# GTEC-UDC/roskfpos

Hardware: AMD Instinct MI355X
Metric: EKF predict+update steps/s at 65536 tags x 8 anchors; RMS pos err vs CPU ref (higher is better)
Workload: dtype f64 arithmetic; f64 state and covariance, f32/int32 measurements in HBM (KFPOS_STORE_MIXED)

## Files before the change

roskfpos_amd/csrc/kfpos_core.h:

```cpp
#ifndef KFPOS_CORE_H
#define KFPOS_CORE_H

#include <math.h>
#include <stdint.h>

#ifndef KFPOS_HD
#define KFPOS_HD
#endif
#define KFPOS_FN KFPOS_HD inline __attribute__((always_inline))
#if defined(__clang__)
#define KFPOS_UNROLL _Pragma("unroll")
#define KFPOS_NOUNROLL _Pragma("nounroll")
#else
#define KFPOS_UNROLL
#define KFPOS_NOUNROLL
#endif

#if defined(__HIP_DEVICE_COMPILE__)
#define KFPOS_WAVE_ALL(pred) (__all((pred) ? 1 : 0) != 0)
#else
#define KFPOS_WAVE_ALL(pred) (pred)
#endif
#if defined(__HIP_DEVICE_COMPILE__)
#define KFPOS_WAVE_ANY(pred) (__builtin_amdgcn_ballot_w64(pred) != 0)
#else
#define KFPOS_WAVE_ANY(pred) (pred)
#endif

namespace kfpos {

enum : uint32_t {
    ST_UPDATE_SKIPPED = 0x01u,
    ST_ML_FALLBACK    = 0x02u,
    ST_FEW_RANGES     = 0x04u,
    ST_ML_INIT        = 0x08u,
    ST_NOT_STARTED    = 0x10u,
    ST_NONFINITE      = 0x20u,
    ST_SKIPPED        = 0x40u,
};
enum : uint32_t { FL_STARTED = 1u, FL_HAS_IMU = 2u };

KFPOS_FN uint32_t pack_status(uint32_t flags, int gain_iters, int ml_iters, int ignored) {
    const uint32_t g = gain_iters > 255 ? 255u : (uint32_t)gain_iters;
    const uint32_t m = ml_iters > 255 ? 255u : (uint32_t)ml_iters;
    return flags | (g << 8) | (m << 16) | ((uint32_t)(ignored + 1) << 24);
}

KFPOS_FN double kf_rcp(double x) {
#if defined(__HIP_DEVICE_COMPILE__)
    double y = __builtin_amdgcn_rcp(x);
    double e = __builtin_fma(-x, y, 1.0);
    y = __builtin_fma(y, e, y);
    e = __builtin_fma(-x, y, 1.0);
    return __builtin_fma(y, e, y);
#else
    return 1.0 / x;
#endif
}
KFPOS_FN double kf_fma(double a, double b, double c) {
#if defined(__HIP_DEVICE_COMPILE__)
    return __builtin_fma(a, b, c);
#else
    return a * b + c;
#endif
}
KFPOS_FN int kf_opaque_zero() {
    int z = 0;
#if defined(__HIP_DEVICE_COMPILE__)
    asm volatile("" : "+v"(z));
#endif
    return z;
}
KFPOS_FN void kf_pin(double &v) {
#if defined(__HIP_DEVICE_COMPILE__)
    asm volatile("" : "+v"(v));
#else
    (void)v;
#endif
}
KFPOS_FN int kf_ctz64(uint64_t m) {
#if defined(__HIP_DEVICE_COMPILE__)
    return __ffsll((unsigned long long)m) - 1;
#else
    return __builtin_ctzll(m);
#endif
}
KFPOS_FN double kf_rsqrt(double x) {
#if defined(__HIP_DEVICE_COMPILE__)
    double y = __builtin_amdgcn_rsq(x);
    const double h = 0.5 * x;
    double e = __builtin_fma(-h * y, y, 0.5);
    y = __builtin_fma(y, e, y);
    e = __builtin_fma(-h * y, y, 0.5);
    return __builtin_fma(y, e, y);
#else
    return 1.0 / sqrt(x);
#endif
}
KFPOS_FN void kf_sqrt_rsqrt(double x, double &d, double &invd) {
#if defined(__HIP_DEVICE_COMPILE__)
    invd = kf_rsqrt(x);
    const double s = x * invd;
    d = __builtin_fma(__builtin_fma(-s, s, x) * 0.5, invd, s);
#else
    d = sqrt(x);
    invd = 1.0 / d;
#endif
}

KFPOS_FN void kf_sqrt_rsqrt_sweep(double x, double &d, double &invd) {
#if defined(__HIP_DEVICE_COMPILE__)
    double y = __builtin_amdgcn_rsq(x);
    const double e = __builtin_fma(-(0.5 * x) * y, y, 0.5);
    y = __builtin_fma(y, e, y);
    const double s = x * y;
    d = __builtin_fma(__builtin_fma(-s, s, x) * 0.5, y, s);
    invd = y;
#else
    d = sqrt(x);
    invd = 1.0 / d;
#endif
}

KFPOS_FN double kf_mm_to_m(int32_t mm) {
#if defined(__HIP_DEVICE_COMPILE__)
    const double x = (double)mm;
    const double q = x * 0.001;
    const double r = __builtin_fma(-q, 1000.0, x);
    return __builtin_fma(r, 0.001, q);
#else
    return (double)mm / 1000;
#endif
}

KFPOS_FN bool rel_change_below(double cost, double c, double tol) {
    const double lhs = fabs(cost - c), rhs = tol * cost;
    const bool clear = cost > 0.0 && fabs(lhs - rhs) > 1e-13 * rhs;
    if (KFPOS_WAVE_ALL(clear)) return lhs < rhs;
    return lhs / cost < tol;
}

KFPOS_FN bool rel_change_below_voted(double cost, double c, double tol) {
    const double lhs = fabs(cost - c), rhs = tol * cost;
    const bool clear = cost > 0.0 && fabs(lhs - rhs) > 1e-13 * rhs;
    bool below = lhs < rhs;
    if (KFPOS_WAVE_ANY(!clear)) below = lhs / cost < tol;
    return below;
}

KFPOS_FN bool rel_change_above(double cost, double c, double tol) {
    const double lhs = fabs(cost - c), rhs = tol * cost;
    const bool clear = cost > 0.0 && fabs(lhs - rhs) > 1e-13 * rhs;
    if (KFPOS_WAVE_ALL(clear)) return lhs > rhs;
    return lhs / cost > tol;
}

KFPOS_FN double stdmax(double a, double b) { return (a < b) ? b : a; }

template <int N, bool SYMM>
struct Cov {
    static constexpr int SZ = SYMM ? N * (N + 1) / 2 : N * N;
    double a[SZ];
    KFPOS_HD static constexpr int idx(int i, int j) {
        return SYMM ? (i <= j ? i * N - i * (i - 1) / 2 + (j - i) : j * N - j * (j - 1) / 2 + (i - j))
                    : i * N + j;
    }
    KFPOS_HD double operator()(int i, int j) const { return a[idx(i, j)]; }
    KFPOS_HD double &operator()(int i, int j) { return a[idx(i, j)]; }
};

struct Params {
    const double *anchors;
    int n_anchors;
    double accel_noise, jolt, cost_threshold;
    int ignore_worst, top_n, use_init_pos;
    int ml_variant = 0;
    int use_fixed_height, imu_fixed_cov_acc, imu_fixed_cov_w;
    double px4_height, px4_arm_p1, px4_arm_p2, px4_cov_vel, px4_cov_gyro_z;
    double imu_cov_acc, imu_cov_w, mag_offset, mag_cov;
    const double *pair_anchor_tab = nullptr;
    bool pair9 = false;
};

KFPOS_FN double sym3_cofactors(const double h[6], double c[6]) {
    c[0] = h[3] * h[5] - h[4] * h[4];
    c[1] = h[2] * h[4] - h[1] * h[5];
    c[2] = h[1] * h[4] - h[2] * h[3];
    c[3] = h[0] * h[5] - h[2] * h[2];
    c[4] = h[1] * h[2] - h[0] * h[4];
    c[5] = h[0] * h[3] - h[1] * h[1];
    return h[0] * c[0] + h[1] * c[1] + h[2] * c[2];
}
KFPOS_FN double gen3_adjugate(const double m[9], double adj[9]) {
    adj[0] = m[4] * m[8] - m[5] * m[7];
    adj[1] = m[2] * m[7] - m[1] * m[8];
    adj[2] = m[1] * m[5] - m[2] * m[4];
    adj[3] = m[5] * m[6] - m[3] * m[8];
    adj[4] = m[0] * m[8] - m[2] * m[6];
    adj[5] = m[2] * m[3] - m[0] * m[5];
    adj[6] = m[3] * m[7] - m[4] * m[6];
    adj[7] = m[1] * m[6] - m[0] * m[7];
    adj[8] = m[0] * m[4] - m[1] * m[3];
    return m[0] * adj[0] + m[1] * adj[3] + m[2] * adj[6];
}

template <int N, int K>
KFPOS_FN void gauss_solve(const double *a, const double *b, double *x) {
    double r[N][N + K];
    KFPOS_UNROLL
    for (int i = 0; i < N; ++i) {
        KFPOS_UNROLL
        for (int j = 0; j < N; ++j) r[i][j] = a[N * i + j];
        KFPOS_UNROLL
        for (int k = 0; k < K; ++k) r[i][N + k] = b[K * i + k];
    }
    KFPOS_UNROLL
    for (int c = 0; c < N; ++c) {
        KFPOS_UNROLL
        for (int i = c + 1; i < N; ++i) {
            const bool sw = fabs(r[i][c]) > fabs(r[c][c]);
            KFPOS_UNROLL
            for (int k = c; k < N + K; ++k) {
                const double tc = r[c][k], ti = r[i][k];
                r[c][k] = sw ? ti : tc;
                r[i][k] = sw ? tc : ti;
            }
        }
        const double ip = 1.0 / r[c][c];
        KFPOS_UNROLL
        for (int i = c + 1; i < N; ++i) {
            const double f = r[i][c] * ip;
            KFPOS_UNROLL
            for (int k = c + 1; k < N + K; ++k) r[i][k] -= f * r[c][k];
        }
// ... 47 lines not shown
    KFPOS_HD void setW(int a, double v) { w[a * stride] = v; }
    KFPOS_HD double Rdyn(int a) const { return r[a * stride]; }
    KFPOS_HD double Edyn(int a) const { return e[a * stride]; }
    KFPOS_HD void setWdyn(int a, double v) { w[a * stride] = v; }
};
template <int N>
struct StaticScratch : Scratch {
    static constexpr int NA = N;
    static constexpr int CHUNK = N > 8 ? 8 : 0;
};
template <int N>
struct StaticScratchF {
    static constexpr int NA = N;
    static constexpr int CHUNK = N > 8 ? 8 : 0;
    static constexpr bool COOP = false;
    double *r, *w;
    float *e;
    int stride;
    KFPOS_HD double R(int a) const { return r[a * stride]; }
    KFPOS_HD double E(int a) const { return (double)e[a * stride]; }
    KFPOS_HD double W(int a) const { return w[a * stride]; }
    KFPOS_HD void setW(int a, double v) { w[a * stride] = v; }
    KFPOS_HD double Rdyn(int a) const { return r[a * stride]; }
    KFPOS_HD double Edyn(int a) const { return (double)e[a * stride]; }
    KFPOS_HD void setWdyn(int a, double v) { w[a * stride] = v; }
};
template <int N>
struct RegScratch {
    static constexpr int NA = N;
    static constexpr int CHUNK = 0;
    static constexpr bool COOP = false;
    double r[N], e[N], w[N];
    KFPOS_HD double R(int a) const { return r[a]; }
    KFPOS_HD double E(int a) const { return e[a]; }
    KFPOS_HD double W(int a) const { return w[a]; }
    KFPOS_HD void setW(int a, double v) { w[a] = v; }
    KFPOS_HD double Rdyn(int a) const {
        double v = 0.0;
        KFPOS_UNROLL
        for (int k = 0; k < N; ++k) v = (k == a) ? r[k] : v;
        return v;
    }
    KFPOS_HD double Edyn(int a) const {
        double v = 1.0;
        KFPOS_UNROLL
        for (int k = 0; k < N; ++k) v = (k == a) ? e[k] : v;
        return v;
    }
    KFPOS_HD void setWdyn(int a, double v) {
        KFPOS_UNROLL
        for (int k = 0; k < N; ++k) w[k] = (k == a) ? v : w[k];
    }
};
struct CoopScratch {
    static constexpr int NA = 1;
    static constexpr int CHUNK = 0;
    static constexpr bool COOP = true;
    double r, e, w;
    double bx, by, bz;
    KFPOS_HD double R(int) const { return r; }
    KFPOS_HD double E(int) const { return e; }
    KFPOS_HD double W(int) const { return w; }
    KFPOS_HD void setW(int, double v) { w = v; }
    KFPOS_HD double Rdyn(int) const { return 0.0; }
    KFPOS_HD double Edyn(int) const { return 1.0; }
    KFPOS_HD void setWdyn(int, double) {}
};

template <class SC>
KFPOS_FN void anchor_of(const SC &sc, const Params &pr, int a, double &bx, double &by, double &bz) {
    if constexpr (SC::COOP) {
        bx = sc.bx; by = sc.by; bz = sc.bz;
    } else {
        bx = pr.anchors[3 * a]; by = pr.anchors[3 * a + 1]; bz = pr.anchors[3 * a + 2];
    }
}

#if defined(__HIP_DEVICE_COMPILE__)
KFPOS_FN double dpp_exchange(double v, int ctrl_tag) {
    const int lo = __double2loint(v), hi = __double2hiint(v);
    int plo, phi;
    if (ctrl_tag == 0) {
        plo = __builtin_amdgcn_mov_dpp(lo, 0xB1, 0xF, 0xF, true);
        phi = __builtin_amdgcn_mov_dpp(hi, 0xB1, 0xF, 0xF, true);
    } else if (ctrl_tag == 1) {
        plo = __builtin_amdgcn_mov_dpp(lo, 0x4E, 0xF, 0xF, true);
        phi = __builtin_amdgcn_mov_dpp(hi, 0x4E, 0xF, 0xF, true);
    } else {
        plo = __builtin_amdgcn_mov_dpp(lo, 0x141, 0xF, 0xF, true);
        phi = __builtin_amdgcn_mov_dpp(hi, 0x141, 0xF, 0xF, true);
    }
    return __hiloint2double(phi, plo);
}
#endif
template <class SC>
KFPOS_FN double group_sum(const SC &, double v) {
    if constexpr (SC::COOP) {
#if defined(__HIP_DEVICE_COMPILE__)
        v += dpp_exchange(v, 0);
        v += dpp_exchange(v, 1);
        v += dpp_exchange(v, 2);
#endif
    }
    return v;
}

// ... 36 lines not shown
```

roskfpos_amd/csrc/kfpos_core_imu9.h:

```cpp
#ifndef KFPOS_CORE_IMU9_H
#define KFPOS_CORE_IMU9_H

namespace kfpos {

constexpr double INFO_FORM_MIN_PIVOT = 1e-7;

struct Tag9 {
    double pos[3], vel[3];
    Cov<9, true> P;
};
struct Imu {
    bool has;
    double acc[3];
    double *ci;
    int ci_stride;
    KFPOS_HD double Wi(int k) const { return ci[(6 + k) * ci_stride]; }
};

KFPOS_FN void imu_whitener(const double s[9], double *ci, int ci_stride) {
    double c00, c11, c22, i00, i11, i22;
    kf_sqrt_rsqrt(s[0], c00, i00);
    const double c10 = s[3] * i00, c20 = s[6] * i00;
    kf_sqrt_rsqrt(s[4] - c10 * c10, c11, i11);
    const double c21 = (s[7] - c20 * c10) * i11;
    kf_sqrt_rsqrt(s[8] - c20 * c20 - c21 * c21, c22, i22);
    const double i10 = -c10 * i00 * i11;
    const double i21 = -c21 * i11 * i22;
    const double i20 = -(c20 * i00 + c21 * i10) * i22;
    ci[0] = i00; ci[ci_stride] = i10; ci[2 * ci_stride] = i20; ci[3 * ci_stride] = i11; ci[4 * ci_stride] = i21;
    ci[5 * ci_stride] = i22;
    double *wi = ci + 6 * ci_stride;
    wi[0] = i00 * i00 + i10 * i10 + i20 * i20;
    wi[ci_stride] = i10 * i11 + i20 * i21;
    wi[2 * ci_stride] = i20 * i22;
    wi[3 * ci_stride] = i11 * i11 + i21 * i21;
    wi[4 * ci_stride] = i21 * i22;
    wi[5 * ci_stride] = i22 * i22;
}

KFPOS_FN void predict9(Cov<9, true> &P, double t, double jolt) {
    const double c = t * t / 2;
    KFPOS_UNROLL
    for (int i = 0; i < 3; ++i) {
        KFPOS_UNROLL
        for (int j = i; j < 3; ++j) {
            const double xpp = P(i, j) + t * P(3 + i, j) + c * P(6 + i, j);
            const double xpv = P(i, 3 + j) + t * P(3 + i, 3 + j) + c * P(6 + i, 3 + j);
            const double xpa = P(i, 6 + j) + t * P(3 + i, 6 + j) + c * P(6 + i, 6 + j);
            P(i, j) = xpp + t * xpv + c * xpa;
        }
    }
    KFPOS_UNROLL
    for (int i = 0; i < 3; ++i) {
        KFPOS_UNROLL
        for (int j = 0; j < 3; ++j) {
            const double xpv = P(i, 3 + j) + t * P(3 + i, 3 + j) + c * P(6 + i, 3 + j);
            const double xpa = P(i, 6 + j) + t * P(3 + i, 6 + j) + c * P(6 + i, 6 + j);
            P(i, 3 + j) = xpv + t * xpa;
        }
    }
    KFPOS_UNROLL
    for (int i = 0; i < 3; ++i) {
        KFPOS_UNROLL
        for (int j = 0; j < 3; ++j) P(i, 6 + j) = P(i, 6 + j) + t * P(3 + i, 6 + j) + c * P(6 + i, 6 + j);
    }
    KFPOS_UNROLL
    for (int i = 0; i < 3; ++i) {
        KFPOS_UNROLL
        for (int j = i; j < 3; ++j) {
// ... 548 lines not shown
        iekf9_sweep4(p, r4, w4, bb, sw);
        other.c = dpp_exchange(sw.c, 0);
        KFPOS_UNROLL
        for (int k = 0; k < 6; ++k) other.m[k] = dpp_exchange(sw.m[k], 0);
        KFPOS_UNROLL
        for (int k = 0; k < 3; ++k) other.u[k] = dpp_exchange(sw.u[k], 0);
        sweep9_add(sw, other);
        iekf9_spread_reads();
        const bool more = iekf9_pass<DIAG, false>(xh, pk, ci, tol, sw, ct, co);
        act = more && co.gain_iters < max_steps;
    }
    const bool owner = (m >> lane) & 1ull;
    const int rank = __popcll(m & ((1ull << lane) - 1ull));
    const int from4 = (owner ? 2 * rank : lane) << 2;
    KFPOS_UNROLL
    for (int k = 0; k < 6; ++k) {
        const double a = lane_pull(ct.wl[k], from4), b = lane_pull(co.mrlast[k], from4);
        if (owner) { it.wl[k] = a; o.mrlast[k] = b; }
    }
    KFPOS_UNROLL
    for (int k = 0; k < 3; ++k) {
        const double a = lane_pull(co.dlast[k], from4);
        if (owner) o.dlast[k] = a;
    }
    const double cst = lane_pull(ct.cost, from4);
    const int gi = __builtin_amdgcn_ds_bpermute(from4, co.gain_iters);
    if (owner) { it.cost = cst; o.gain_iters = gi; }
}
template <bool DIAG, bool ALLIMU, bool ACC0>
KFPOS_FN void iekf9_pairs_held(uint64_t m, const double xhat[9], const double *binv, int binv_stride,
                               const RegScratch<8> &sc, const Params &pr, const Imu &imu, int max_steps, double tol,
                               Iekf9Iter &it, Iekf9Out &o) {
    const int lane = (int)__builtin_amdgcn_mbcnt_hi(~0u, __builtin_amdgcn_mbcnt_lo(~0u, 0u));
    const int g = lane >> 1;
    const bool h = lane & 1;
    const int n_surv = __popcll(m);
    bool act = g < n_surv;
    const int src = nth_set_bit(m, act ? g : 0);
    const int src4 = src << 2;
    Imu ci;
    ci.ci = imu.ci + (src - lane);
    ci.ci_stride = imu.ci_stride;
    Iekf9Parked pk;
    iekf9_fetch<false, DIAG, false>(binv + (src - lane), binv_stride, ci, pk);
    double xh[9];
    KFPOS_UNROLL
    for (int k = 0; k < 3; ++k) {
        xh[k] = lane_pull(xhat[k], src4);
        xh[3 + k] = 0.0;
        xh[6 + k] = ACC0 ? 0.0 : lane_pull(xhat[6 + k], src4);
    }
    Iekf9Iter ct;
    KFPOS_UNROLL
    for (int k = 0; k < 6; ++k) { ct.ve[k] = lane_pull(it.ve[k], src4); ct.wl[k] = 0.0; }
    ct.qd = lane_pull(it.qd, src4);
    ct.cost = lane_pull(it.cost, src4);
    Iekf9Out co;
    KFPOS_UNROLL
    for (int k = 0; k < 6; ++k) co.mrlast[k] = 0.0;
    KFPOS_UNROLL
    for (int k = 0; k < 3; ++k) co.dlast[k] = 0.0;
    co.gain_iters = __builtin_amdgcn_ds_bpermute(src4, o.gain_iters);
    ci.has = ALLIMU || __builtin_amdgcn_ds_bpermute(src4, imu.has ? 1 : 0) != 0;
    KFPOS_UNROLL
    for (int k = 0; k < 3; ++k) ci.acc[k] = lane_pull(imu.acc[k], src4);
    double r4[4], w4[4], bb[12];
    KFPOS_UNROLL
    for (int k = 0; k < 4; ++k) {
        const double r0 = lane_pull(sc.r[k], src4), r1 = lane_pull(sc.r[4 + k], src4);
        const double w0 = lane_pull(sc.w[k], src4), w1 = lane_pull(sc.w[4 + k], src4);
        r4[k] = h ? r1 : r0;
        w4[k] = h ? w1 : w0;
    }
    KFPOS_UNROLL
    for (int k = 0; k < 12; ++k) {
        bb[k] = h ? pr.anchors[12 + k] : pr.anchors[k];
        kf_pin(bb[k]);
    }
    KFPOS_UNROLL
    for (int k = 0; k < 21; ++k) kf_pin(pk.binv[k]);
    KFPOS_UNROLL
    for (int k = 0; k < 6; ++k) {
        if (!DIAG || k == 0 || k == 3 || k == 5) kf_pin(pk.wi[k]);
    }
    __builtin_amdgcn_s_waitcnt(0xC07F);
    while (act) {
        const double p[3] = {xh[0] + ct.ve[0], xh[1] + ct.ve[1], xh[2] + ct.ve[2]};
        Sweep9 sw, other;
        iekf9_sweep4(p, r4, w4, bb, sw);
        other.c = dpp_exchange(sw.c, 0);
        KFPOS_UNROLL
        for (int k = 0; k < 6; ++k) other.m[k] = dpp_exchange(sw.m[k], 0);
        KFPOS_UNROLL
        for (int k = 0; k < 3; ++k) other.u[k] = dpp_exchange(sw.u[k], 0);
        sweep9_add(sw, other);
        const bool more = iekf9_pass<DIAG, ALLIMU>(xh, pk, ci, tol, sw, ct, co);
        act = more && co.gain_iters < max_steps;
    }
    const bool owner = (m >> lane) & 1ull;
    const int rank = __popcll(m & ((1ull << lane) - 1ull));
    const int from4 = (owner ? 2 * rank : lane) << 2;
    const int gi = __builtin_amdgcn_ds_bpermute(from4, co.gain_iters);
    double back[16];
    KFPOS_UNROLL
    for (int k = 0; k < 6; ++k) { back[k] = lane_pull(ct.wl[k], from4); back[6 + k] = lane_pull(co.mrlast[k], from4); }
    KFPOS_UNROLL
    for (int k = 0; k < 3; ++k) back[12 + k] = lane_pull(co.dlast[k], from4);
    back[15] = lane_pull(ct.cost, from4);
    const bool moved = owner & (gi != o.gain_iters);
    KFPOS_UNROLL
    for (int k = 0; k < 6; ++k) { it.wl[k] = moved ? back[k] : it.wl[k]; o.mrlast[k] = moved ? back[6 + k] : o.mrlast[k]; }
    KFPOS_UNROLL
    for (int k = 0; k < 3; ++k) o.dlast[k] = moved ? back[12 + k] : o.dlast[k];
    it.cost = moved ? back[15] : it.cost;
    o.gain_iters = moved ? gi : o.gain_iters;
}
#endif

template <bool DIAG, bool ALLIMU, bool RANGING, bool ACC0 = false, bool HOLD = true, bool SETTLE = false,
          bool TAIL = false, class SC>
KFPOS_FN void iekf9_info(const double xhat[9], const double *binv, int binv_stride, SC &sc, const Params &pr,
                         const Imu &imu, int max_steps, double tol, Iekf9Out &o) {
    Iekf9Iter it;
    KFPOS_UNROLL
    for (int k = 0; k < 6; ++k) { it.ve[k] = 0.0; it.wl[k] = 0.0; o.mrlast[k] = 0.0; }
    it.qd = 0.0;
    it.cost = 1e20;
    o.dlast[0] = o.dlast[1] = o.dlast[2] = 0.0;
    o.gain_iters = 0;
// ... 283 lines not shown
```

roskfpos_amd/csrc/kfpos_core_ml.h:

```cpp
#ifndef KFPOS_CORE_ML_H
#define KFPOS_CORE_ML_H

namespace kfpos {

template <class SC>
KFPOS_FN void ml_sweep(const double p[3], const SC &sc, const Params &pr, uint64_t drop,
                              double &cw, double &sse, double g[3], double hs[6]) {
    double cw_ = 0.0, sse_ = 0.0, g0 = 0.0, g1 = 0.0, g2 = 0.0, c0s = 0.0;
    double h0 = 0.0, h1 = 0.0, h2 = 0.0, h3 = 0.0, h4 = 0.0, h5 = 0.0;
    for_anchors<SC>(pr, [&](int a) {
        const bool on = used(sc, a, drop);
        const double r = sc.R(a), w = sc.W(a);
        double bx, by, bz;
        anchor_of(sc, pr, a, bx, by, bz);
        const double dx = bx - p[0], dy = by - p[1], dz = bz - p[2];
        double d, invd;
        kf_sqrt_rsqrt_sweep(dx * dx + dy * dy + dz * dz, d, invd);
        const double rd = r - d, rd2 = rd * rd;
        cw_ += rd2 * w;
        sse_ += on ? rd2 : 0.0;
        const double wi = w * invd, gi = rd * wi, wq = r * wi;
        g0 += gi * dx;
        g1 += gi * dy;
        g2 += gi * dz;
// ... 91 lines not shown
}

template <class SC>
KFPOS_FN int ml_estimate(double p[3], const SC &sc, const Params &pr, uint64_t drop, int n_used, double &sse_out) {
    MlFirst unused = {};
    return ml_estimate(p, sc, pr, drop, n_used, sse_out, false, unused, false, unused);
}

template <class SC>
KFPOS_FN bool ml_covariance(const double p[3], const SC &sc, const Params &pr, double sse,
                                   double cov[6]) {
    double m0 = 0, m1 = 0, m2 = 0, m3 = 0, m4 = 0, m5 = 0, c[6];
    for_anchors<SC>(pr, [&](int a) {
        if (!used(sc, a, 0)) return;
        double bx, by, bz;
        anchor_of(sc, pr, a, bx, by, bz);
        const double dx = p[0] - bx, dy = p[1] - by, dz = p[2] - bz;
        const double invd = 1.0 / sqrt(dx * dx + dy * dy + dz * dz);
        const double w = 1.0 / stdmax(sc.E(a), sse);
        const double gx = dx * invd, gy = dy * invd, gz = dz * invd;
        m0 += w * gx * gx; m1 += w * gx * gy; m2 += w * gx * gz;
        m3 += w * gy * gy; m4 += w * gy * gz; m5 += w * gz * gz;
    });
    const double m[6] = {group_sum(sc, m0), group_sum(sc, m1), group_sum(sc, m2),
                         group_sum(sc, m3), group_sum(sc, m4), group_sum(sc, m5)};
    const double det = sym3_cofactors(m, c);
    const double idet = 1.0 / det;
    KFPOS_UNROLL
    for (int k = 0; k < 6; ++k) cov[k] = c[k] * idet;
    return det != 0.0;
}

template <bool SELECTS = true, class SC>
KFPOS_FN bool ml_covariance_throws(const SC &sc, const Params &pr, uint64_t drop, int n_used, double sse,
                                   int min_used = 4) {
    if (n_used < min_used) return false;
    bool bad = false;
    if constexpr (SC::COOP || !SELECTS) {
        for_anchors<SC>(pr, [&](int a) { bad = bad || (used(sc, a, drop) && stdmax(sc.E(a), sse) == 0.0); });
        if constexpr (SC::COOP) bad = group_sum(sc, bad ? 1.0 : 0.0) > 0.0;
    } else {
        for_anchors<SC>(pr, [&](int a) {
            const bool on = used(sc, a, drop), zero = stdmax(sc.E(a), sse) == 0.0;
            bad = bad | (on & zero);
        });
    }
    return bad;
}

template <bool SELECTS = true, class SC>
KFPOS_FN void set_weights_ml(SC &sc, const Params &pr, uint64_t drop) {
    if constexpr (SC::COOP || !SELECTS) {
        for_anchors<SC>(pr, [&](int a) { sc.setW(a, used(sc, a, drop) ? kf_rcp(sc.E(a)) : 0.0); });
        return;
    }
    for_anchors<SC>(pr, [&](int a) {
        const double rcp = kf_rcp(sc.E(a));
        sc.setW(a, used(sc, a, drop) ? rcp : 0.0);
    });
}
template <bool SELECTS = true, class SC>
KFPOS_FN void set_weights_iekf(SC &sc, const Params &pr, double e_ml, uint64_t drop) {
    if constexpr (SC::COOP) {
        sc.setW(0, used(sc, 0, drop) ? kf_rcp(stdmax(e_ml, sc.E(0))) : 0.0);
        return;
    }
    const double r_ml = kf_rcp(e_ml);
    if constexpr (!SELECTS) {
        for_anchors<SC>(pr, [&](int a) { sc.setW(a, used(sc, a, drop) ? ((e_ml < sc.E(a)) ? sc.W(a) : r_ml) : 0.0); });
        return;
    }
    for_anchors<SC>(pr, [&](int a) {
        const bool on = used(sc, a, drop), own = on & (e_ml < sc.E(a));
        const double w_own = sc.W(a);
        const double w = own ? w_own : r_ml;
        sc.setW(a, on ? w : 0.0);
    });
}

template <bool SHARE, class SC>
KFPOS_FN uint64_t topn_mask(const double seed[3], SC &sc, const Params &pr, int n_valid, MlFirst &first_all,
                            bool &first_valid, bool &weights_kept, int *rank_iters = nullptr) {
    weights_kept = false;
    first_valid = false;
    if (rank_iters) *rank_iters = 0;
    int ndrop = n_valid - 4 < pr.top_n ? n_valid - 4 : pr.top_n;
    if (ndrop <= 0) return 0;
    first_valid = SHARE;
    double p[3] = {seed[0], seed[1], seed[2]}, sse;
    set_weights_ml(sc, pr, 0ull);
    MlFirst unused = {};
    const int it_rank = ml_estimate(p, sc, pr, 0, n_valid, sse, false, unused, SHARE, first_all);
    if (rank_iters) *rank_iters = it_rank;
    uint64_t drop = 0;
    if (SHARE && ndrop <= 2) {
        double v1 = -1.0, v2 = -1.0;
        int i1 = -1, i2 = -1;
        for_anchors<SC>(pr, [&](int a) {
            const double dx = pr.anchors[3 * a] - p[0], dy = pr.anchors[3 * a + 1] - p[1], dz = pr.anchors[3 * a + 2] - p[2];
            double d, invd;
            kf_sqrt_rsqrt(dx * dx + dy * dy + dz * dz, d, invd);
            const double rd = d - sc.R(a);
            const double r2 = used(sc, a, 0) ? rd * rd : -1.0;
            const bool first = r2 > v1, second = !first && r2 > v2;
            v2 = first ? v1 : (second ? r2 : v2);
            i2 = first ? i1 : (second ? a : i2);
// ... 143 lines not shown
```

roskfpos_amd/csrc/kfpos_k_imu9.hip:

```cpp
#include "kfpos_kernels.h"

namespace {

template <typename W>
__device__ inline void in_agpr(W &w) {
    static_assert(sizeof(W) == 4, "one register");
    asm volatile("" : "+a"(w));
}

__device__ inline void forget(double &v) { asm volatile("" : "=v"(v)); }

template <typename REAL, typename MREAL, int AS, bool RANGING = true>
__global__ __launch_bounds__(WAVE) void k_step_imu9(const KArgs a) {
    extern __shared__ double lds[];
    const int lane = threadIdx.x;
    const size_t t = (size_t)blockIdx.x * WAVE + lane;
    if (t >= (size_t)a.T) return;
    const size_t T = a.T;
    const uint32_t t32 = (uint32_t)t;
    Params pr = make_params(a);
    constexpr bool has_ranging = RANGING;
    constexpr bool AHEAD = sizeof(MREAL) == 4 && !std::is_same<REAL, float>::value;
    const bool fresh_imu = a.mode != MODE_TOA;
    constexpr int NA = AS > 0 ? AS : 1;
    double dt_tag = a.dt_shared;
    if (a.n_steps == 1 && a.dt) {
        dt_tag = a.dt[t32];
        if (dt_tag < 0.0) {
            skipped_lane(a, t, true);
            return;
        }
    }

    uint32_t fl = a.flags[t32];
    RawEpoch<MREAL, NA> raw;
    RawImu<MREAL> rawi;
    if constexpr (AS > 0) {
        if (has_ranging) fetch_epoch<MREAL, AS>(a, t, 0, raw);
    }
    Tag9 tg;
#pragma unroll
    for (int k = 0; k < 3; ++k) {
        tg.pos[k] = (a.pos + k * T)[t32];
        tg.vel[k] = (a.vel + k * T)[t32];
    }
    const CovPark9 park{lds + ((AS == 0 && has_ranging) ? 3 * (size_t)a.A * WAVE : 0) + lane, WAVE};
    Imu imu;
    imu.has = false;
    imu.ci = park.a + 66 * WAVE;
    imu.ci_stride = WAVE;
    constexpr bool TAIL = AS == 8 && RANGING && sizeof(MREAL) == 4 && !std::is_same<REAL, float>::value;
    if constexpr (TAIL) pr.pair9 = a.pair9 != 0;
    else if constexpr (AS == 8 && RANGING) {
        if (a.pair9) {
            double *tab = lds + 78 * WAVE;
#pragma unroll
            for (int k = 0; k < 24; ++k) tab[k] = a.anchors[k];
            pr.pair_anchor_tab = tab;
        }
    }
    double cv[9] = {1, 0, 0, 0, 1, 0, 0, 0, 1};
    MREAL rawc[9];
    if (fresh_imu) {
        fetch_imu<MREAL>(a, t, 0, rawi);
        fetch_imu_cov<MREAL>(a, t, 0, rawc);
    } else if (fl & FL_HAS_IMU) {
        imu.has = true;
#pragma unroll
        for (int k = 0; k < 3; ++k) imu.acc[k] = ldrow<MREAL>(a.imu_acc, k, T, t32);
        cv[0] = ldrow<MREAL>(a.imu_cov, 0, T, t32);
        cv[3] = ldrow<MREAL>(a.imu_cov, 1, T, t32);
        cv[4] = ldrow<MREAL>(a.imu_cov, 2, T, t32);
        cv[6] = ldrow<MREAL>(a.imu_cov, 3, T, t32);
        cv[7] = ldrow<MREAL>(a.imu_cov, 4, T, t32);
        cv[8] = ldrow<MREAL>(a.imu_cov, 5, T, t32);
    }
#pragma unroll
    for (int k = 0; k < 45; ++k) tg.P.a[k] = ldcov<REAL>(a.P, k, 45, T, t32);
    if (fresh_imu) {
        imu.has = true;
#pragma unroll
        for (int k = 0; k < 9; ++k) cv[k] = (double)rawc[k];
        if (a.latch) latch_imu_cov<MREAL>(a, T, t32, cv);
    }
    if (imu.has) imu_whitener(cv, imu.ci, imu.ci_stride);
    bool diag = false;
    if (a.imu9_diag) {
        const bool mine = !imu.has || (imu.Wi(1) == 0.0 && imu.Wi(2) == 0.0 && imu.Wi(4) == 0.0);
        diag = __builtin_amdgcn_ballot_w64(mine) == __builtin_amdgcn_ballot_w64(true);
    }
    const bool fast = imu9_fast(diag, imu.has);

    const bool multi = a.n_steps > 1;
    double dt_next = multi ? a.dt_steps[0] : dt_tag;
    constexpr bool IMU_WITH_EPOCH = AHEAD && AS > 0 && RANGING;
    constexpr bool ROTATE = IMU_WITH_EPOCH && AS == 8 && std::is_same<REAL, double>::value;

    __builtin_amdgcn_s_waitcnt(0x0F70);
    uint32_t s = 0;
    if constexpr (ROTATE) {
        bool invertible = step_imu9_head(tg, pr, dt_next, park);
        double latched[3] = {0.0, 0.0, 0.0};
        if (!fresh_imu && imu.has) {
#pragma unroll
            for (int k = 0; k < 3; ++k) latched[k] = imu.acc[k];
        }
        for (int e = 0; e < a.n_steps; ++e) {
            const double dt = dt_next;
            const bool more = e + 1 < a.n_steps;
            if (multi && more) dt_next = a.dt_steps[opaque_uniform(e + 1)];
#pragma unroll
            for (int k = 0; k < NA; ++k) { in_agpr(raw.mm[k]); in_agpr(raw.e[k]); }
            if (fresh_imu) {
#pragma unroll
                for (int k = 0; k < 3; ++k) in_agpr(rawi.acc[k]);
            }
#pragma unroll
            for (int k = 0; k < 3; ++k) imu.acc[k] = fresh_imu ? (double)rawi.acc[k] : latched[k];
            RegScratch<NA> sc;
            unpack_epoch<MREAL, NA>(raw, sc);
#pragma unroll
            for (int k = 0; k < NA; ++k) { kfpos::kf_pin(sc.r[k]); kfpos::kf_pin(sc.e[k]); }
#pragma unroll
            for (int k = 0; k < 3; ++k) kfpos::kf_pin(imu.acc[k]);
            asm volatile("" ::: "memory");
            const int ahead = opaque_uniform(more ? e + 1 : e);
            fetch_epoch<MREAL, NA>(a, opaque_lane(t), ahead, raw);
            if (fresh_imu) fetch_imu<MREAL>(a, opaque_lane(t), ahead, rawi);
            Iekf9Out o;
#pragma unroll
            for (int k = 0; k < 6; ++k) { forget(o.w[k]); forget(o.mrlast[k]); }
#pragma unroll
            for (int k = 0; k < 3; ++k) forget(o.dlast[k]);
            const bool update = step_imu9_state_parked<RANGING, true, TAIL>(tg, sc, pr, dt, imu, park, fast, invertible, o, s);
            if (a.traj) {
#pragma unroll
                for (int k = 0; k < 3; ++k) (a.traj + ((size_t)opaque_uniform(e) * 3 + k) * T)[t32] = tg.pos[k];
            }
            if (update) s = step_imu9_cov(tg, o, imu);
            if (more) {
                static_assert(!cov_is_rounded<REAL>(), "a rounded covariance is rounded here, in front of the head");
                invertible = step_imu9_head(tg, pr, dt_next, park);
#pragma unroll
                for (int k = 0; k < 45; ++k) forget(tg.P.a[k]);
            }
        }
    } else
    for (int e = 0; e < a.n_steps; ++e) {
        const double dt = dt_next;
        if (multi && e + 1 < a.n_steps) dt_next = a.dt_steps[opaque_uniform(e + 1)];
        if (fresh_imu) {
#pragma unroll
            for (int k = 0; k < 3; ++k) imu.acc[k] = (double)rawi.acc[k];
            if constexpr (AHEAD && !IMU_WITH_EPOCH) {
                if (e + 1 < a.n_steps) fetch_imu<MREAL>(a, opaque_lane(t), opaque_uniform(e + 1), rawi);
            }
        }
        Iekf9Out o;
        auto finish = [&](bool update) {
            if (a.traj) {
#pragma unroll
                for (int k = 0; k < 3; ++k) (a.traj + ((size_t)opaque_uniform(e) * 3 + k) * T)[t32] = tg.pos[k];
            }
            if (update) s = step_imu9_cov(tg, o, imu);
        };
        if constexpr (AS > 0) {
            RegScratch<AS> sc;
            if (has_ranging) {
                unpack_epoch<MREAL, AS>(raw, sc);
                if (e + 1 < a.n_steps) {
                    if constexpr (AHEAD) {
                        fetch_epoch<MREAL, AS>(a, opaque_lane(t), opaque_uniform(e + 1), raw);
                        if constexpr (IMU_WITH_EPOCH) {
                            if (fresh_imu) fetch_imu<MREAL>(a, opaque_lane(t), opaque_uniform(e + 1), rawi);
                        }
                    }
                }
            } else {
#pragma unroll
                for (int k = 0; k < AS; ++k) sc.r[k] = sc.e[k] = sc.w[k] = 0.0;
            }
            finish(step_imu9_state<RANGING, true, TAIL>(tg, sc, pr, dt, imu, park, fast, o, s));
            if constexpr (!AHEAD) {
                if (e + 1 < a.n_steps) {
                    if (fresh_imu) fetch_imu<MREAL>(a, opaque_lane(t), opaque_uniform(e + 1), rawi);
                    if (has_ranging) fetch_epoch<MREAL, AS>(a, opaque_lane(t), opaque_uniform(e + 1), raw);
                }
            }
        } else {
            Scratch sc{nullptr, nullptr, nullptr, WAVE};
            if (has_ranging) sc = stage_epoch_lds<MREAL>(a, lds, lane, t, opaque_uniform(e));
            finish(step_imu9_state<RANGING, true, TAIL>(tg, sc, pr, dt, imu, park, fast, o, s));
            if constexpr (!AHEAD) {
                if (e + 1 < a.n_steps && fresh_imu) fetch_imu<MREAL>(a, opaque_lane(t), opaque_uniform(e + 1), rawi);
            }
        }
        if constexpr (cov_is_rounded<REAL>()) {
            if (e + 1 < a.n_steps) {
#pragma unroll
                for (int k = 0; k < 45; ++k) tg.P.a[k] = round_cov<REAL>(tg.P.a[k]);
            }
        }
    }

    if (fresh_imu && a.latch) {
#pragma unroll
        for (int k = 0; k < 3; ++k) strow<MREAL>(a.imu_acc, k, T, t32, imu.acc[k]);
        fl |= FL_HAS_IMU;
    }
    bool fin = true;
#pragma unroll
    for (int k = 0; k < 3; ++k) {
        (a.pos + k * T)[t32] = tg.pos[k];
        (a.vel + k * T)[t32] = tg.vel[k];
        fin &= isfinite(tg.pos[k]) & isfinite(tg.vel[k]);
    }
#pragma unroll
    for (int k = 0; k < 45; ++k) {
        stcov<REAL>(a.P, k, 45, T, t32, tg.P.a[k]);
        fin &= isfinite(tg.P.a[k]);
    }
    const bool waiting = !a.use_init_pos && isnan(tg.pos[0]);
    if (!fin && !waiting) s |= ST_NONFINITE;
    a.flags[t32] = fl | FL_STARTED;
    if (a.status) a.status[t32] = s;
// ... 14 lines not shown
```

roskfpos_amd/csrc/kfpos_kernels.h:

```cpp
#ifndef KFPOS_KERNELS_H
#define KFPOS_KERNELS_H

#include <hip/hip_runtime.h>

#include <cmath>
#include <cstdint>
#include <cstring>
#include <type_traits>

#define KFPOS_HD __host__ __device__
#include "kfpos_core.h"
#include "kfpos_internal.h"
#include "kfpos_launch_plan.h"
#include "kfpos_p48.h"
#include "kfpos_replay_plan.h"
#include "kfpos_state_record.h"

namespace kfpos_k {

struct KArgs {
    double anchors[KFPOS_MAX_ANCHORS * 3];
    int T, A;
    double accel_noise, jolt, cost_threshold;
    int ignore_worst, top_n, use_init_pos, ml_variant;
// ... 335 lines not shown
        (void)rows;
        (((REAL *)p) + row * T)[t] = (REAL)v;
    }
}
#define KFPOS_BY_STORAGE(st, F, ...)                                                                          \
    ((st) == KFPOS_STORE_F32 ? F<float, float>(__VA_ARGS__)                                                   \
     : (st) == KFPOS_STORE_MIXED ? F<double, float>(__VA_ARGS__)                                              \
     : (st) == KFPOS_STORE_P48 ? F<p48, float>(__VA_ARGS__) : F<double, double>(__VA_ARGS__))

template <class P>
__device__ inline P make_params_of(const KArgs &a) {
    P pr;
    pr.anchors = a.anchors;
    pr.n_anchors = a.A;
    pr.accel_noise = a.accel_noise;
    pr.jolt = a.jolt;
    pr.cost_threshold = a.cost_threshold;
    pr.ignore_worst = a.ignore_worst;
    pr.top_n = a.top_n;
    pr.ml_variant = a.ml_variant;
    pr.use_init_pos = a.use_init_pos;
    pr.use_fixed_height = a.use_fixed_height;
    pr.imu_fixed_cov_acc = a.imu_fixed_cov_acc;
    pr.imu_fixed_cov_w = a.imu_fixed_cov_w;
    pr.px4_height = a.px4_height;
    pr.px4_arm_p1 = a.px4_arm_p1;
    pr.px4_arm_p2 = a.px4_arm_p2;
    pr.px4_cov_vel = a.px4_cov_vel;
    pr.px4_cov_gyro_z = a.px4_cov_gyro_z;
    pr.imu_cov_acc = a.imu_cov_acc;
    pr.imu_cov_w = a.imu_cov_w;
    pr.mag_offset = a.mag_offset;
    pr.mag_cov = a.mag_cov;
    return pr;
}
__device__ inline Params make_params(const KArgs &a) { return make_params_of<Params>(a); }

template <typename MREAL, int AS>
struct RawEpoch {
    int32_t mm[AS];
    MREAL e[AS];
};
template <typename MREAL, int AS>
__device__ inline void fetch_epoch(const KArgs &a, size_t t, int s, RawEpoch<MREAL, AS> &raw) {
    const int32_t *rp = a.ranges + (size_t)s * a.stride_ranges;
    const MREAL *ep = (const MREAL *)a.err + (size_t)s * a.stride_err;
#pragma unroll
    for (int k = 0; k < AS; ++k) {
        raw.mm[k] = (rp + (size_t)k * a.T)[(uint32_t)t];
        raw.e[k] = (ep + (size_t)k * a.T)[(uint32_t)t];
    }
}
template <typename MREAL, int AS>
__device__ inline void unpack_epoch(const RawEpoch<MREAL, AS> &raw, RegScratch<AS> &sc) {
#pragma unroll
    for (int k = 0; k < AS; ++k) {
        sc.r[k] = raw.mm[k] > 0 ? kf_mm_to_m(raw.mm[k]) : 0.0;
        sc.e[k] = (double)raw.e[k];
        sc.w[k] = 0.0;
    }
}
template <typename MREAL>
__device__ inline Scratch stage_epoch_lds(const KArgs &a, double *lds, int lane, size_t t, int s) {
    Scratch sc;
    sc.r = lds + lane;
    sc.e = lds + (size_t)a.A * WAVE + lane;
    sc.w = lds + 2 * (size_t)a.A * WAVE + lane;
    sc.stride = WAVE;
    const int32_t *rp = a.ranges + (size_t)s * a.stride_ranges;
    const MREAL *ep = (const MREAL *)a.err + (size_t)s * a.stride_err;
    for (int k = 0; k < a.A; ++k) {
        const int32_t mm = (rp + (size_t)k * a.T)[(uint32_t)t];
        sc.r[k * WAVE] = mm > 0 ? kf_mm_to_m(mm) : 0.0;
        sc.e[k * WAVE] = (double)(ep + (size_t)k * a.T)[(uint32_t)t];
    }
    return sc;
}
template <typename MREAL, int N>
__device__ inline StaticScratch<N> stage_epoch_lds_n(const KArgs &a, double *lds, int lane, size_t t, int s) {
    StaticScratch<N> sc;
    sc.r = lds + lane;
    sc.e = lds + (size_t)N * WAVE + lane;
    sc.w = lds + 2 * (size_t)N * WAVE + lane;
    sc.stride = WAVE;
    RawEpoch<MREAL, N> raw;
    fetch_epoch<MREAL, N>(a, t, s, raw);
#pragma unroll
    for (int k = 0; k < N; ++k) {
        sc.r[k * WAVE] = raw.mm[k] > 0 ? kf_mm_to_m(raw.mm[k]) : 0.0;
        sc.e[k * WAVE] = (double)raw.e[k];
    }
    return sc;
}
template <typename MREAL>
struct RawImu {
    MREAL acc[3];
};
template <typename MREAL>
__device__ inline void fetch_imu(const KArgs &a, size_t t, int s, RawImu<MREAL> &raw) {
    const MREAL *ap = (const MREAL *)a.accel + (size_t)s * a.stride_accel;
#pragma unroll
    for (int k = 0; k < 3; ++k) raw.acc[k] = (ap + (size_t)k * a.T)[(uint32_t)t];
}
template <typename MREAL>
__device__ inline void fetch_imu_cov(const KArgs &a, size_t t, int s, MREAL raw[9]) {
    const MREAL *cp = (const MREAL *)a.cov + (size_t)s * a.stride_cov;
// ... 59 lines not shown
```

Baseline: 2.268 billion.

## Hoist held measurement errors and reciprocals out of epoch loop; slim pair-tail lane traffic

When the per-epoch error array has zero stride, the errors and their reciprocal weights are computed once before the time loop and reused, and only range words are fetched each epoch. The pair-tail path now shuffles IMU acceleration as 32-bit floats instead of doubles and takes per-lane anchor coordinates precomputed into a params struct. Dead initialisations are replaced with an asm 'forget' so the compiler emits no zeroing moves. This trims loads, reciprocals and cross-lane permutes per step, at the cost of extra live registers for the held values.

```diff
diff --git a/roskfpos_amd/csrc/kfpos_core.h b/roskfpos_amd/csrc/kfpos_core.h
--- a/roskfpos_amd/csrc/kfpos_core.h
+++ b/roskfpos_amd/csrc/kfpos_core.h
@@ -74,6 +74,13 @@
 KFPOS_FN void kf_pin(double &v) {
 #if defined(__HIP_DEVICE_COMPILE__)
     asm volatile("" : "+v"(v));
+#else
+    (void)v;
+#endif
+}
+KFPOS_FN void kf_forget(double &v) {
+#if defined(__HIP_DEVICE_COMPILE__)
+    asm volatile("" : "=v"(v));
 #else
     (void)v;
 #endif
@@ -180,6 +187,9 @@
     double imu_cov_acc, imu_cov_w, mag_offset, mag_cov;
     const double *pair_anchor_tab = nullptr;
     bool pair9 = false;
+};
+struct ParamsPairs : Params {
+    double pair_bb[12];
 };
 
 KFPOS_FN double sym3_cofactors(const double h[6], double c[6]) {
@@ -333,6 +343,18 @@
         for (int k = 0; k < N; ++k) w[k] = (k == a) ? v : w[k];
     }
 };
+template <int N>
+struct RegScratchRcp : RegScratch<N> {
+    double rw[N];
+};
+template <class SC>
+struct holds_rcp {
+    static constexpr bool value = false;
+};
+template <int N>
+struct holds_rcp<RegScratchRcp<N>> {
+    static constexpr bool value = true;
+};
 struct CoopScratch {
     static constexpr int NA = 1;
     static constexpr int CHUNK = 0;
diff --git a/roskfpos_amd/csrc/kfpos_core_imu9.h b/roskfpos_amd/csrc/kfpos_core_imu9.h
--- a/roskfpos_amd/csrc/kfpos_core_imu9.h
+++ b/roskfpos_amd/csrc/kfpos_core_imu9.h
@@ -15,6 +15,9 @@
     double *ci;
     int ci_stride;
     KFPOS_HD double Wi(int k) const { return ci[(6 + k) * ci_stride]; }
+};
+struct ImuPairs : Imu {
+    float acc32[3];
 };
 
 KFPOS_FN void imu_whitener(const double s[9], double *ci, int ci_stride) {
@@ -669,18 +672,21 @@
     }
     Iekf9Iter ct;
     KFPOS_UNROLL
-    for (int k = 0; k < 6; ++k) { ct.ve[k] = lane_pull(it.ve[k], src4); ct.wl[k] = 0.0; }
+    for (int k = 0; k < 6; ++k) { ct.ve[k] = lane_pull(it.ve[k], src4); kf_forget(ct.wl[k]); }
     ct.qd = lane_pull(it.qd, src4);
     ct.cost = lane_pull(it.cost, src4);
     Iekf9Out co;
     KFPOS_UNROLL
-    for (int k = 0; k < 6; ++k) co.mrlast[k] = 0.0;
-    KFPOS_UNROLL
-    for (int k = 0; k < 3; ++k) co.dlast[k] = 0.0;
+    for (int k = 0; k < 6; ++k) kf_forget(co.mrlast[k]);
+    KFPOS_UNROLL
+    for (int k = 0; k < 3; ++k) kf_forget(co.dlast[k]);
     co.gain_iters = __builtin_amdgcn_ds_bpermute(src4, o.gain_iters);
     ci.has = ALLIMU || __builtin_amdgcn_ds_bpermute(src4, imu.has ? 1 : 0) != 0;
     KFPOS_UNROLL
-    for (int k = 0; k < 3; ++k) ci.acc[k] = lane_pull(imu.acc[k], src4);
+    for (int k = 0; k < 3; ++k) {
+        const float a32 = static_cast<const ImuPairs &>(imu).acc32[k];
+        ci.acc[k] = (double)__int_as_float(__builtin_amdgcn_ds_bpermute(src4, __float_as_int(a32)));
+    }
     double r4[4], w4[4], bb[12];
     KFPOS_UNROLL
     for (int k = 0; k < 4; ++k) {
@@ -691,7 +697,7 @@
     }
     KFPOS_UNROLL
     for (int k = 0; k < 12; ++k) {
-        bb[k] = h ? pr.anchors[12 + k] : pr.anchors[k];
+        bb[k] = static_cast<const ParamsPairs &>(pr).pair_bb[k];
         kf_pin(bb[k]);
     }
     KFPOS_UNROLL
diff --git a/roskfpos_amd/csrc/kfpos_core_ml.h b/roskfpos_amd/csrc/kfpos_core_ml.h
--- a/roskfpos_amd/csrc/kfpos_core_ml.h
+++ b/roskfpos_amd/csrc/kfpos_core_ml.h
@@ -167,6 +167,10 @@
 KFPOS_FN void set_weights_ml(SC &sc, const Params &pr, uint64_t drop) {
     if constexpr (SC::COOP || !SELECTS) {
         for_anchors<SC>(pr, [&](int a) { sc.setW(a, used(sc, a, drop) ? kf_rcp(sc.E(a)) : 0.0); });
+        return;
+    }
+    if constexpr (holds_rcp<SC>::value) {
+        for_anchors<SC>(pr, [&](int a) { sc.setW(a, used(sc, a, drop) ? sc.rw[a] : 0.0); });
         return;
     }
     for_anchors<SC>(pr, [&](int a) {
diff --git a/roskfpos_amd/csrc/kfpos_k_imu9.hip b/roskfpos_amd/csrc/kfpos_k_imu9.hip
--- a/roskfpos_amd/csrc/kfpos_k_imu9.hip
+++ b/roskfpos_amd/csrc/kfpos_k_imu9.hip
@@ -18,7 +18,9 @@
     if (t >= (size_t)a.T) return;
     const size_t T = a.T;
     const uint32_t t32 = (uint32_t)t;
-    Params pr = make_params(a);
+    constexpr bool TAIL = AS == 8 && RANGING && sizeof(MREAL) == 4 && !std::is_same<REAL, float>::value;
+    typename std::conditional<TAIL, ParamsPairs, Params>::type pr;
+    static_cast<Params &>(pr) = make_params(a);
     constexpr bool has_ranging = RANGING;
     constexpr bool AHEAD = sizeof(MREAL) == 4 && !std::is_same<REAL, float>::value;
     const bool fresh_imu = a.mode != MODE_TOA;
@@ -35,6 +37,7 @@
     uint32_t fl = a.flags[t32];
     RawEpoch<MREAL, NA> raw;
     RawImu<MREAL> rawi;
+    MREAL acc_latched[3] = {0, 0, 0};
     if constexpr (AS > 0) {
         if (has_ranging) fetch_epoch<MREAL, AS>(a, t, 0, raw);
     }
@@ -45,13 +48,18 @@
         tg.vel[k] = (a.vel + k * T)[t32];
     }
     const CovPark9 park{lds + ((AS == 0 && has_ranging) ? 3 * (size_t)a.A * WAVE : 0) + lane, WAVE};
-    Imu imu;
+    typename std::conditional<TAIL, ImuPairs, Imu>::type imu;
     imu.has = false;
     imu.ci = park.a + 66 * WAVE;
     imu.ci_stride = WAVE;
-    constexpr bool TAIL = AS == 8 && RANGING && sizeof(MREAL) == 4 && !std::is_same<REAL, float>::value;
-    if constexpr (TAIL) pr.pair9 = a.pair9 != 0;
-    else if constexpr (AS == 8 && RANGING) {
+    if constexpr (TAIL) {
+        pr.pair9 = a.pair9 != 0;
+        if (pr.pair9) {
+            const bool odd = lane & 1;
+#pragma unroll
+            for (int k = 0; k < 12; ++k) pr.pair_bb[k] = odd ? a.anchors[12 + k] : a.anchors[k];
+        }
+    } else if constexpr (AS == 8 && RANGING) {
         if (a.pair9) {
             double *tab = lds + 78 * WAVE;
 #pragma unroll
@@ -67,7 +75,11 @@
     } else if (fl & FL_HAS_IMU) {
         imu.has = true;
 #pragma unroll
-        for (int k = 0; k < 3; ++k) imu.acc[k] = ldrow<MREAL>(a.imu_acc, k, T, t32);
+        for (int k = 0; k < 3; ++k) {
+            acc_latched[k] = (((const MREAL *)a.imu_acc) + (size_t)k * T)[t32];
+            imu.acc[k] = (double)acc_latched[k];
+            if constexpr (TAIL) imu.acc32[k] = acc_latched[k];
+        }
         cv[0] = ldrow<MREAL>(a.imu_cov, 0, T, t32);
         cv[3] = ldrow<MREAL>(a.imu_cov, 1, T, t32);
         cv[4] = ldrow<MREAL>(a.imu_cov, 2, T, t32);
@@ -98,34 +110,73 @@
 
     __builtin_amdgcn_s_waitcnt(0x0F70);
     uint32_t s = 0;
+    using Sc = typename std::conditional<TAIL, RegScratchRcp<NA>, RegScratch<NA>>::type;
+    const bool held_err = TAIL && multi && a.stride_err == 0;
+    double he[NA], hw[NA];
+    if constexpr (TAIL) {
+        if (held_err) {
+#pragma unroll
+            for (int k = 0; k < NA; ++k) {
+                he[k] = (double)raw.e[k];
+                hw[k] = kfpos::kf_rcp(he[k]);
+            }
+        } else {
+#pragma unroll
+            for (int k = 0; k < NA; ++k) { forget(he[k]); forget(hw[k]); }
+        }
+    }
+    auto errs_of_epoch = [&](Sc &sc) {
+        if constexpr (TAIL) {
+            if (!held_err) {
+#pragma unroll
+                for (int k = 0; k < NA; ++k) {
+                    he[k] = sc.e[k];
+                    if constexpr (ROTATE) kfpos::kf_pin(he[k]);
+                    hw[k] = kfpos::kf_rcp(he[k]);
+                }
+            }
+#pragma unroll
+            for (int k = 0; k < NA; ++k) { sc.e[k] = he[k]; sc.rw[k] = hw[k]; }
+        }
+    };
     if constexpr (ROTATE) {
         bool invertible = step_imu9_head(tg, pr, dt_next, park);
-        double latched[3] = {0.0, 0.0, 0.0};
+        static_assert(TAIL && sizeof(MREAL) == 4, "the sample is a 4-byte word, fresh or latched");
+        float latched[3] = {0.0f, 0.0f, 0.0f};
         if (!fresh_imu && imu.has) {
 #pragma unroll
-            for (int k = 0; k < 3; ++k) latched[k] = imu.acc[k];
+            for (int k = 0; k < 3; ++k) latched[k] = acc_latched[k];
         }
         for (int e = 0; e < a.n_steps; ++e) {
             const double dt = dt_next;
             const bool more = e + 1 < a.n_steps;
             if (multi && more) dt_next = a.dt_steps[opaque_uniform(e + 1)];
 #pragma unroll
-            for (int k = 0; k < NA; ++k) { in_agpr(raw.mm[k]); in_agpr(raw.e[k]); }
+            for (int k = 0; k < NA; ++k) in_agpr(raw.mm[k]);
+            if (!held_err) {
+#pragma unroll
+                for (int k = 0; k < NA; ++k) in_agpr(raw.e[k]);
+            }
             if (fresh_imu) {
 #pragma unroll
                 for (int k = 0; k < 3; ++k) in_agpr(rawi.acc[k]);
             }
 #pragma unroll
-            for (int k = 0; k < 3; ++k) imu.acc[k] = fresh_imu ? (double)rawi.acc[k] : latched[k];
-            RegScratch<NA> sc;
+            for (int k = 0; k < 3; ++k) {
+                imu.acc32[k] = fresh_imu ? rawi.acc[k] : latched[k];
+                imu.acc[k] = (double)imu.acc32[k];
+            }
+            Sc sc;
             unpack_epoch<MREAL, NA>(raw, sc);
 #pragma unroll
-            for (int k = 0; k < NA; ++k) { kfpos::kf_pin(sc.r[k]); kfpos::kf_pin(sc.e[k]); }
+            for (int k = 0; k < NA; ++k) kfpos::kf_pin(sc.r[k]);
+            errs_of_epoch(sc);
 #pragma unroll
             for (int k = 0; k < 3; ++k) kfpos::kf_pin(imu.acc[k]);
             asm volatile("" ::: "memory");
             const int ahead = opaque_uniform(more ? e + 1 : e);
-            fetch_epoch<MREAL, NA>(a, opaque_lane(t), ahead, raw);
+            fetch_epoch_ranges<MREAL, NA>(a, opaque_lane(t), ahead, raw);
+            if (!held_err) fetch_epoch_errs<MREAL, NA>(a, opaque_lane(t), ahead, raw);
             if (fresh_imu) fetch_imu<MREAL>(a, opaque_lane(t), ahead, rawi);
             Iekf9Out o;
 #pragma unroll
@@ -151,7 +202,10 @@
         if (multi && e + 1 < a.n_steps) dt_next = a.dt_steps[opaque_uniform(e + 1)];
         if (fresh_imu) {
 #pragma unroll
-            for (int k = 0; k < 3; ++k) imu.acc[k] = (double)rawi.acc[k];
+            for (int k = 0; k < 3; ++k) {
+                imu.acc[k] = (double)rawi.acc[k];
+                if constexpr (TAIL) imu.acc32[k] = rawi.acc[k];
+            }
             if constexpr (AHEAD && !IMU_WITH_EPOCH) {
                 if (e + 1 < a.n_steps) fetch_imu<MREAL>(a, opaque_lane(t), opaque_uniform(e + 1), rawi);
             }
@@ -165,12 +219,18 @@
             if (update) s = step_imu9_cov(tg, o, imu);
         };
         if constexpr (AS > 0) {
-            RegScratch<AS> sc;
+            Sc sc;
             if (has_ranging) {
                 unpack_epoch<MREAL, AS>(raw, sc);
+                errs_of_epoch(sc);
                 if (e + 1 < a.n_steps) {
                     if constexpr (AHEAD) {
-                        fetch_epoch<MREAL, AS>(a, opaque_lane(t), opaque_uniform(e + 1), raw);
+                        if constexpr (TAIL) {
+                            fetch_epoch_ranges<MREAL, AS>(a, opaque_lane(t), opaque_uniform(e + 1), raw);
+                            if (!held_err) fetch_epoch_errs<MREAL, AS>(a, opaque_lane(t), opaque_uniform(e + 1), raw);
+                        } else {
+                            fetch_epoch<MREAL, AS>(a, opaque_lane(t), opaque_uniform(e + 1), raw);
+                        }
                         if constexpr (IMU_WITH_EPOCH) {
                             if (fresh_imu) fetch_imu<MREAL>(a, opaque_lane(t), opaque_uniform(e + 1), rawi);
                         }
diff --git a/roskfpos_amd/csrc/kfpos_kernels.h b/roskfpos_amd/csrc/kfpos_kernels.h
--- a/roskfpos_amd/csrc/kfpos_kernels.h
+++ b/roskfpos_amd/csrc/kfpos_kernels.h
@@ -411,6 +411,18 @@
     }
 }
 template <typename MREAL, int AS>
+__device__ inline void fetch_epoch_ranges(const KArgs &a, size_t t, int s, RawEpoch<MREAL, AS> &raw) {
+    const int32_t *rp = a.ranges + (size_t)s * a.stride_ranges;
+#pragma unroll
+    for (int k = 0; k < AS; ++k) raw.mm[k] = (rp + (size_t)k * a.T)[(uint32_t)t];
+}
+template <typename MREAL, int AS>
+__device__ inline void fetch_epoch_errs(const KArgs &a, size_t t, int s, RawEpoch<MREAL, AS> &raw) {
+    const MREAL *ep = (const MREAL *)a.err + (size_t)s * a.stride_err;
+#pragma unroll
+    for (int k = 0; k < AS; ++k) raw.e[k] = (ep + (size_t)k * a.T)[(uint32_t)t];
+}
+template <typename MREAL, int AS>
 __device__ inline void unpack_epoch(const RawEpoch<MREAL, AS> &raw, RegScratch<AS> &sc) {
 #pragma unroll
     for (int k = 0; k < AS; ++k) {
```

Result: no change. 2.281 billion (median of 6 runs) (+0.6%).
